# hongfz16/Garment4D

Hardware: AMD Instinct MI355X
Metric: point-cloud frames/s (FPS+ball_query+SA-MLP+LBS), B=8 N=8192 (higher is better)
Workload: dtype f32

## Files before the change

garment4d_amd/csrc/api.hip:

```cpp
#include <stdarg.h>
#include <stddef.h>
#include <stdlib.h>
#include <string.h>

#include "mlp_common.h"

namespace g4d {
static thread_local char g_err[512] = "";

void set_error(const char *fmt, ...) {
    va_list ap;
    va_start(ap, fmt);
    vsnprintf(g_err, sizeof(g_err), fmt, ap);
    va_end(ap);
}

static int g_contract = -1;

static int parse_contract(const char *e) {
    if (!e || !*e) return G4D_CONTRACT_NVCC;
    if (!strcmp(e, "0") || !strcmp(e, "off") || !strcmp(e, "none")) return G4D_CONTRACT_OFF;
    if (!strcmp(e, "2") || !strcmp(e, "chain") || !strcmp(e, "inner")) return G4D_CONTRACT_CHAIN;
    return G4D_CONTRACT_NVCC;
}

static thread_local int t_contract = -1;

int distance_contraction() {
    if (t_contract >= 0) return t_contract;
    int m = __atomic_load_n(&g_contract, __ATOMIC_RELAXED);
    if (m < 0) {
        m = parse_contract(getenv("G4D_DIST_CONTRACT"));
        __atomic_store_n(&g_contract, m, __ATOMIC_RELAXED);
    }
    return m;
}
}

namespace g4d {
namespace {
struct Tune { const char *key; long long value; int state; };
Tune g_tune[] = {{"sa_table_persistent", 0, 0}, {"sa_table_min_rows", 0, 0}, {"sa_table_128", 0, 0}, {"sa_table_oversub", 0, 0}, {"sa_table_dedup", 0, 0}, {"fp_table_persistent", 0, 0},
                 {"fp_table_min_rows", 0, 0}, {"gemm_tile", 0, 0}, {"gemm_tile_min_rows", 0, 0}, {"gemm_tile_min_cout", 0, 0}, {"gemm_tile_min_kpad", 0, 0}, {"fp_init_persistent", 0, 0}, {"fp_init_min_rows", 0, 0},
                 {"fp_head_bf16_persistent", 0, 0}, {"fp_head_bf16_min_rows", 0, 0}, {"sa_group_bf16_persistent", 0, 0}, {"sa_group_bf16_min_rows", 0, 0}};
}
struct ThreadTune { long long value; bool set; };
thread_local ThreadTune t_tune[sizeof(g_tune) / sizeof(g_tune[0])] = {};

long long tuning(const char *key, long long dflt) {
    int i = 0;
    for (Tune &t : g_tune) {
        const int slot = i++;
        if (strcmp(t.key, key)) continue;
        if (t_tune[slot].set) return t_tune[slot].value;
        int st = __atomic_load_n(&t.state, __ATOMIC_ACQUIRE);
        if (st == 0) {
            char env[64] = "G4D_";
            size_t n = 4;
            for (const char *c = key; *c && n + 1 < sizeof(env); ++c) env[n++] = (char)((*c >= 'a' && *c <= 'z') ? *c - 32 : *c);
            env[n] = 0;
            const char *e = getenv(env);
            const long long v = e && *e ? atoll(e) : dflt;
            int expect = 0;
            if (__atomic_compare_exchange_n(&t.state, &expect, 3, false, __ATOMIC_ACQ_REL, __ATOMIC_ACQUIRE)) {
                __atomic_store_n(&t.value, v, __ATOMIC_RELAXED);
                expect = 3;
                __atomic_compare_exchange_n(&t.state, &expect, 1, false, __ATOMIC_ACQ_REL, __ATOMIC_ACQUIRE);
                return v;
            }
            st = expect;
            if (st == 3) return v;
        }
        return __atomic_load_n(&t.value, __ATOMIC_RELAXED);
    }
    return dflt;
}
}

extern "C" int g4d_tuning_set(const char *key, long long value) {
    if (key)
        for (g4d::Tune &t : g4d::g_tune)
            if (!strcmp(t.key, key)) {
                __atomic_store_n(&t.value, value, __ATOMIC_RELAXED);
                __atomic_store_n(&t.state, 2, __ATOMIC_RELEASE);
                return G4D_OK;
            }
    g4d::set_error("g4d_tuning_set: unknown key '%s'", key ? key : "(null)");
    return G4D_EINVAL;
}

extern "C" int g4d_tuning_set_thread(const char *key, long long value, int set) {
    if (key) {
        int i = 0;
        for (g4d::Tune &t : g4d::g_tune) {
            const int slot = i++;
            if (!strcmp(t.key, key)) {
                g4d::t_tune[slot].value = value;
                g4d::t_tune[slot].set = set != 0;
                return G4D_OK;
            }
        }
    }
    g4d::set_error("g4d_tuning_set_thread: unknown key '%s'", key ? key : "(null)");
    return G4D_EINVAL;
}

extern "C" int g4d_version(void) { return 263;  }
extern "C" const char *g4d_last_error(void) { return g4d::g_err; }

extern "C" int g4d_get_distance_contraction(void) { return g4d::distance_contraction(); }
extern "C" int g4d_set_distance_contraction_thread(int mode) {
    const int prev = g4d::t_contract;
    if (mode < -1 || mode > G4D_CONTRACT_CHAIN) {
        g4d::set_error("g4d_set_distance_contraction_thread: mode %d is not -1 (no override) or one of G4D_CONTRACT_OFF/NVCC/CHAIN", mode);
        return -2;
    }
    g4d::t_contract = mode;
    return prev;
}

extern "C" int g4d_set_distance_contraction(int mode) {
    const int saved = g4d::t_contract;
    g4d::t_contract = -1;
    const int prev = g4d::distance_contraction();
    g4d::t_contract = saved;
    if (mode < G4D_CONTRACT_OFF || mode > G4D_CONTRACT_CHAIN) {
        g4d::set_error("g4d_set_distance_contraction: mode %d is not one of G4D_CONTRACT_OFF/NVCC/CHAIN", mode);
        return -1;
    }
    __atomic_store_n(&g4d::g_contract, mode, __ATOMIC_RELAXED);
    return prev;
}

namespace g4d {
struct CopySegs { float *dst[4]; const float *src[4]; long long n[4]; long long first_block[5]; };
__global__ void __launch_bounds__(256) copy_segments_kernel(const CopySegs c, int nseg) {
    int s = 0;
    while (s + 1 < nseg && (long long)blockIdx.x >= c.first_block[s + 1]) ++s;
    const long long i0 = ((long long)blockIdx.x - c.first_block[s]) * 1024 + threadIdx.x * 4;
    float *d = c.dst[s];
    const float *p = c.src[s];
    const long long n = c.n[s];
    if (i0 + 3 < n && ((reinterpret_cast<size_t>(d) | reinterpret_cast<size_t>(p)) & 15) == 0) {
        *reinterpret_cast<float4 *>(d + i0) = *reinterpret_cast<const float4 *>(p + i0);
    } else {
        for (int e = 0; e < 4; ++e)
            if (i0 + e < n) d[i0 + e] = p[i0 + e];
    }
}
}

extern "C" int g4d_copy_segments_f32(int nseg, float *const *dst, const float *const *src, const long long *nfloats, g4d_stream_t stream) {
    G4D_REQUIRE(nseg >= 0 && nseg <= 4 && (nseg == 0 || (dst && src && nfloats)), "g4d_copy_segments_f32: 0..4 segments");
    g4d::CopySegs c = {};
    long long blocks = 0;
    int k = 0;
    for (int i = 0; i < nseg; ++i) {
        G4D_REQUIRE(nfloats[i] >= 0 && (nfloats[i] == 0 || (dst[i] && src[i])), "g4d_copy_segments_f32: bad segment %d", i);
        if (nfloats[i] == 0) continue;
        c.dst[k] = dst[i]; c.src[k] = src[i]; c.n[k] = nfloats[i]; c.first_block[k] = blocks;
        blocks += (nfloats[i] + 1023) / 1024;
        ++k;
    }
    if (k == 0) return G4D_OK;
    c.first_block[k] = blocks;
    G4D_REQUIRE(blocks < (1ll << 31), "g4d_copy_segments_f32: too large");
    hipLaunchKernelGGL(g4d::copy_segments_kernel, dim3((unsigned)blocks), dim3(256), 0, reinterpret_cast<hipStream_t>(stream), c, k);
    return g4d::check_launch("g4d_copy_segments_f32");
}

namespace g4d {
static StackCall stack_call(const char *name, const g4d_mlp_args &a) {
    StackCall c = {};
    c.name = name; c.mode = a.mode; c.rows = a.rows;
    LinearArgs &in = c.in;
    in.K = a.K0; in.out = a.out; in.ldo = a.ldo; in.col0 = a.col0; in.pool = a.pool; in.S = a.S;
    in.X = a.X; in.ldx = a.ldx;
    in.xyz = a.xyz; in.new_xyz = a.new_xyz; in.feats = a.feats; in.idx = a.idx; in.N = a.N; in.P = a.P; in.C = a.C; in.use_xyz = a.use_xyz;
    in.known_feats = a.known_feats; in.skip = a.skip; in.dist2 = a.dist2; in.nn_idx = a.nn_idx; in.C2 = a.C2; in.C1 = a.C1; in.m = a.m; in.n = a.n;
    in.rowptr = a.rowptr; in.colidx = a.colidx; in.vals = a.vals; in.Vg = a.Vg;
    c.nlayers = a.nlayers; c.W = a.W; c.scale = a.scale; c.shift = a.shift; c.Kpad = a.Kpad; c.Cout = a.Cout; c.relu = a.relu;
    c.tap_layer = a.tap_layer; c.tap_out = a.tap_out; c.tap_ld = a.tap_ld; c.unknown_grid = a.unknown_grid;
    return c;
}

int stack_call_check(const StackCall &c, const StackRules &r) {
    const int S = c.in.S, pool = c.in.pool;
    G4D_REQUIRE(c.mode >= 0 && c.mode <= (r.csr ? LOAD_CSR : LOAD_INTERP), "%s: %s", c.name, r.bad_mode);
    if (r.max_layers) G4D_REQUIRE(c.nlayers >= 1 && c.nlayers <= r.max_layers, "%s: 1..%d layers", c.name, r.max_layers);
    G4D_REQUIRE(c.rows >= 0 && c.rows < r.max_rows && c.in.K > 0, "%s: bad sizes", c.name);
    if (c.rows == 0) return kEmptyLaunch;
    G4D_REQUIRE(has_layer_arrays(c), "%s: null pointer", c.name);
    if (!r.max_layers) G4D_REQUIRE(g4d_mlp_chain_supported(c.nlayers, c.Cout), "%s: unsupported layer widths (see g4d_mlp_chain_supported)", c.name);
    G4D_REQUIRE(pool >= 0 && pool <= 2, "%s: pool must be 0|1|2", c.name);
    if (pool) G4D_REQUIRE((S == 4 || S == 8 || S == 16 || S == 32 || S == 64) && c.rows % S == 0, "%s: pooling needs S in {4,8,16,32,64}", c.name);
    for (int l = 0; l < c.nlayers; ++l) {
        const void *const *Wl = c.W + (size_t)l * r.w_pieces;
        G4D_REQUIRE(Wl[0] && (r.w_pieces == 1 || (Wl[1] && Wl[2])) && c.scale[l] && c.shift[l] && c.Kpad[l] % r.kpad_multiple == 0 && c.Cout[l] > 0, "%s: bad layer %d", c.name, l);
    }
    G4D_REQUIRE(tap_layer_of(c) < c.nlayers - 1, "%s: tap must be a hidden layer", c.name);
    return G4D_OK;
}
}

extern "C" unsigned g4d_mlp_args_size(void) { return (unsigned)sizeof(g4d_mlp_args); }

extern "C" int g4d_mlp_run(int family, const g4d_mlp_args *args, g4d_stream_t stream) {
    using namespace g4d;
    G4D_REQUIRE(args, "g4d_mlp_run: null argument block");
    G4D_REQUIRE(args->version == G4D_MLP_ARGS_VERSION, "g4d_mlp_run: argument block version %u, this library speaks %d", args->version, G4D_MLP_ARGS_VERSION);
    G4D_REQUIRE(args->size >= 16 && args->size <= sizeof(g4d_mlp_args), "g4d_mlp_run: argument block of %u bytes, this library's is %u (a newer caller?)",
                args->size, (unsigned)sizeof(g4d_mlp_args));
    g4d_mlp_args a;
    memset(&a, 0, sizeof(a));
    memcpy(&a, args, args->size);
    if (args->size < offsetof(g4d_mlp_args, tap_layer) + sizeof(int)) a.tap_layer = -1;
    if (family != G4D_MLP_CHAIN_BF16) a.unknown_grid = nullptr;
    hipStream_t st = reinterpret_cast<hipStream_t>(stream);
    switch (family) {
        case G4D_MLP_STACK_F32: return mlp_stack_f32_run(stack_call("g4d_mlp_stack_f32", a), st);
        case G4D_MLP_STACK_BF16: return mlp_stack_bf16_run(stack_call("g4d_mlp_stack_bf16", a), st);
        case G4D_MLP_WAVE_F32: return mlp_wave_f32_run(stack_call("g4d_mlp_wave_f32", a), st);
        case G4D_MLP_CHAIN_F32: return mlp_chain_f32_run(stack_call("g4d_mlp_chain_f32", a), st);
        case G4D_MLP_CHAIN_BF16: return mlp_chain_bf16_run(stack_call("g4d_mlp_chain_bf16", a), st);
        case G4D_MLP_CHAIN_BF16X3: return mlp_chain_bf16x3_run(stack_call("g4d_mlp_chain_bf16x3", a), st);
    }
    set_error("g4d_mlp_run: unknown kernel family %d", family);
    return G4D_EINVAL;
}

#define G4D_MLP_LOADERS                                                                                                                       \
    int mode, long long rows, int K0,  const float *X, int ldx,                                                            \
     int N, int P, int S, int C, int use_xyz, const float *xyz, const float *new_xyz, const float *feats, const int *idx,        \
     int n, int m, int C2, int C1, const float *known_feats, const float *skip, const float *dist2, const int *nn_idx
#define G4D_MLP_LAYERS(WT)                                                                                                                    \
    int nlayers, const WT *const *W, const float *const *scale, const float *const *shift, const int *Kpad, const int *Cout, const int *relu, \
     int pool, float *out, int ldo, int col0
#define G4D_MLP_COMMON                                                                                                                        \
    mode, rows, K0, X, ldx, N, P, S, C, use_xyz, xyz, new_xyz, feats, idx, n, m, C2, C1, known_feats, skip, dist2, nn_idx, nlayers,         \
    reinterpret_cast<const void *const *>(W), scale, shift, Kpad, Cout, relu, pool, out, ldo, col0

static g4d_mlp_args pack_args(G4D_MLP_LOADERS, G4D_MLP_LAYERS(void), int tap_layer = -1, float *tap_out = nullptr, int tap_ld = 0) {
    g4d_mlp_args a;
    memset(&a, 0, sizeof(a));
    a.size = (unsigned)sizeof(a); a.version = G4D_MLP_ARGS_VERSION;
    a.mode = mode; a.rows = rows; a.K0 = K0; a.X = X; a.ldx = ldx;
    a.N = N; a.P = P; a.S = S; a.C = C; a.use_xyz = use_xyz; a.xyz = xyz; a.new_xyz = new_xyz; a.feats = feats; a.idx = idx;
    a.n = n; a.m = m; a.C2 = C2; a.C1 = C1; a.known_feats = known_feats; a.skip = skip; a.dist2 = dist2; a.nn_idx = nn_idx;
    a.nlayers = nlayers; a.W = W; a.scale = scale; a.shift = shift; a.Kpad = Kpad; a.Cout = Cout; a.relu = relu;
    a.pool = pool; a.out = out; a.ldo = ldo; a.col0 = col0; a.tap_layer = tap_layer; a.tap_out = tap_out; a.tap_ld = tap_ld;
    return a;
}

extern "C" int g4d_mlp_stack_f32(G4D_MLP_LOADERS,  int Vg, const int *rowptr, const int *colidx, const float *vals, G4D_MLP_LAYERS(float),
                                 int tap_layer, float *tap_out, int tap_ld, g4d_stream_t stream) {
    g4d_mlp_args a = pack_args(G4D_MLP_COMMON, tap_layer, tap_out, tap_ld);
    a.Vg = Vg; a.rowptr = rowptr; a.colidx = colidx; a.vals = vals;
    return g4d_mlp_run(G4D_MLP_STACK_F32, &a, stream);
}

extern "C" int g4d_mlp_stack_bf16(G4D_MLP_LOADERS,  int Vg, const int *rowptr, const int *colidx, const float *vals, G4D_MLP_LAYERS(unsigned short),
                                  int tap_layer, float *tap_out, int tap_ld, g4d_stream_t stream) {
    g4d_mlp_args a = pack_args(G4D_MLP_COMMON, tap_layer, tap_out, tap_ld);
    a.Vg = Vg; a.rowptr = rowptr; a.colidx = colidx; a.vals = vals;
    return g4d_mlp_run(G4D_MLP_STACK_BF16, &a, stream);
}

extern "C" int g4d_mlp_wave_f32(G4D_MLP_LOADERS,  int Vg, const int *rowptr, const int *colidx, const float *vals, G4D_MLP_LAYERS(float),
                                g4d_stream_t stream) {
    g4d_mlp_args a = pack_args(G4D_MLP_COMMON);
    a.Vg = Vg; a.rowptr = rowptr; a.colidx = colidx; a.vals = vals;
    return g4d_mlp_run(G4D_MLP_WAVE_F32, &a, stream);
}

extern "C" int g4d_mlp_chain_f32(G4D_MLP_LOADERS, G4D_MLP_LAYERS(float), int tap_layer, float *tap_out, int tap_ld, g4d_stream_t stream) {
    g4d_mlp_args a = pack_args(G4D_MLP_COMMON, tap_layer, tap_out, tap_ld);
    return g4d_mlp_run(G4D_MLP_CHAIN_F32, &a, stream);
}

extern "C" int g4d_mlp_chain_bf16(G4D_MLP_LOADERS, G4D_MLP_LAYERS(unsigned short), int tap_layer, float *tap_out, int tap_ld, g4d_stream_t stream) {
    g4d_mlp_args a = pack_args(G4D_MLP_COMMON, tap_layer, tap_out, tap_ld);
    return g4d_mlp_run(G4D_MLP_CHAIN_BF16, &a, stream);
}

extern "C" int g4d_mlp_chain_cells_bf16(G4D_MLP_LOADERS, G4D_MLP_LAYERS(unsigned short), int tap_layer, float *tap_out, int tap_ld, const void *unknown_grid,
                                        g4d_stream_t stream) {
    g4d_mlp_args a = pack_args(G4D_MLP_COMMON, tap_layer, tap_out, tap_ld);
    a.unknown_grid = unknown_grid;
    return g4d_mlp_run(G4D_MLP_CHAIN_BF16, &a, stream);
}

extern "C" int g4d_mlp_chain_bf16x3(G4D_MLP_LOADERS, G4D_MLP_LAYERS(unsigned short), int tap_layer, float *tap_out, int tap_ld, g4d_stream_t stream) {
    g4d_mlp_args a = pack_args(G4D_MLP_COMMON, tap_layer, tap_out, tap_ld);
    return g4d_mlp_run(G4D_MLP_CHAIN_BF16X3, &a, stream);
}
```

garment4d_amd/csrc/fps.hip:

```cpp
#include "g4d_common.h"

namespace g4d {

template <int U>
__device__ __host__ constexpr int brev_small(int v) {
    int r = 0;
    for (int bit = 1, rb = U >> 1; bit < U; bit <<= 1, rb >>= 1)
        if (v & bit) r |= rb;
    return r;
}

__device__ __forceinline__ float min_f32(float a, float b) {
    float r;
    asm("v_min_f32 %0, %1, %2" : "=v"(r) : "v"(a), "v"(b));
    return r;
}

struct FpsCand {
    float val;
    unsigned rank;
    int k;
    int pad;
};

__device__ __forceinline__ unsigned fps_rank(int k, int bs, int log2bs) {
    const unsigned c = (unsigned)k & (unsigned)(bs - 1);
    const unsigned q = (unsigned)k >> log2bs;
    const unsigned br = log2bs ? (__builtin_bitreverse32(c) >> (32 - log2bs)) : 0u;
    return (br << 16) | q;
}

template <int W>
__device__ __forceinline__ unsigned long long row_max_u64(unsigned long long key) {
#define G4D_STEP(CTRL)                                                                                       \
    {                                                                                                        \
        const unsigned lo = (unsigned)__builtin_amdgcn_update_dpp(0, (int)(unsigned)key, CTRL, 0xf, 0xf, true);        \
        const unsigned hi = (unsigned)__builtin_amdgcn_update_dpp(0, (int)(unsigned)(key >> 32), CTRL, 0xf, 0xf, true); \
        const unsigned long long o = ((unsigned long long)hi << 32) | lo;                                    \
        key = o > key ? o : key;                                                                             \
    }
    G4D_STEP(0x111)
    G4D_STEP(0x112)
    if constexpr (W >= 8) G4D_STEP(0x114)
    if constexpr (W >= 16) G4D_STEP(0x118)
#undef G4D_STEP
    return key;
}

__device__ __forceinline__ void wave_argmax(float best, int k, int bs, int log2bs, float &wval, int &wk, unsigned &wrank) {
    wval = wave_max_f32(best);
    const unsigned long long hit = __builtin_amdgcn_ballot_w64(best == wval);
    int lane;
    if (__builtin_popcountll(hit) == 1) {
        lane = __builtin_ctzll(hit);
        wk = __builtin_amdgcn_readlane(k, lane);
        wrank = fps_rank(wk, bs, log2bs);
    } else {
        const unsigned r = (best == wval) ? fps_rank(k, bs, log2bs) : 0xffffffffu;
        wrank = wave_min_u32(r);
        lane = __builtin_ctzll(__builtin_amdgcn_ballot_w64(r == wrank));
        wk = __builtin_amdgcn_readlane(k, lane);
    }
}

template <int W, int U, int Q, int FM>
__global__ void __launch_bounds__(64 * W) fps_reg_kernel(int n, int m, int bs, int log2bs, const float *__restrict__ xyz_all,
                                                        float *__restrict__ temp_all, int *__restrict__ idx_all, float *__restrict__ nx_all) {
    constexpr int T = 64 * W, P = U * Q;
    extern __shared__ __attribute__((aligned(16))) unsigned char smem_raw[];
    float *sx = reinterpret_cast<float *>(smem_raw + 2 * 16 * 16);
    float *sy = sx + n;
    float *sz = sy + n;
    int *spick = reinterpret_cast<int *>(sz + n);

    const int t = threadIdx.x;
    const float *xyz = xyz_all + (size_t)blockIdx.x * n * 3;
    float *temp = temp_all + (size_t)blockIdx.x * n;
    int *idx = idx_all + (size_t)blockIdx.x * m;
    float *nx = nx_all ? nx_all + (size_t)blockIdx.x * m * 3 : nullptr;

    float px[P], py[P], pz[P], md[P];
#pragma unroll
    for (int i = 0; i < P; ++i) {
        const int k = t + brev_small<U>(i / Q) * T + (i % Q) * bs;
        const bool ok = k < n;
        px[i] = ok ? xyz[k * 3 + 0] : 0.f;
        py[i] = ok ? xyz[k * 3 + 1] : 0.f;
        pz[i] = ok ? xyz[k * 3 + 2] : 0.f;
        md[i] = ok ? (temp_all ? temp[k] : 1e10f) : -2.f;
        if (ok) { sx[k] = px[i]; sy[k] = py[i]; sz[k] = pz[i]; }
    }
    if (t == 0) spick[0] = 0;
    __syncthreads();

    float x1 = sx[0], y1 = sy[0], z1 = sz[0];
    const int wave = t >> 6;
    for (int j = 1; j < m; ++j) {
        float best = -1.f;
        int bslot = 0;
#pragma unroll
        for (int i = 0; i < P; ++i) {
            const float dx = px[i] - x1, dy = py[i] - y1, dz = pz[i] - z1;
            const float d = dist2<FM>(dx, dy, dz);
            const float d2 = min_f32(d, md[i]);
            md[i] = d2;
            const bool gt = d2 > best;
            bslot = gt ? i : bslot;
            best = gt ? d2 : best;
        }
        int k;
        if constexpr (P == 1) k = t;
        else k = t + brev_small<U>(bslot / Q) * T + (bslot % Q) * bs;
        float wval; int wk; unsigned wrank;
        wave_argmax(best, k, bs, log2bs, wval, wk, wrank);
        int old;
        if constexpr (W == 1) {
            old = wk;
        } else {
            unsigned long long *buf = reinterpret_cast<unsigned long long *>(smem_raw) + (j & 1) * 16;
            if ((t & 63) == 0)
                buf[wave] = ((unsigned long long)__float_as_uint(fmaxf(wval, 0.f)) << 32) | (unsigned)(~wrank);
            __syncthreads();
            const unsigned long long key = row_max_u64<W>(buf[t & (W - 1)]);
            const unsigned rank = ~(unsigned)__builtin_amdgcn_readlane((int)(unsigned)key, W - 1);
            const unsigned c = log2bs ? (__builtin_bitreverse32(rank >> 16) >> (32 - log2bs)) : 0u;
            old = (int)(((rank & 0xffffu) << log2bs) | c);
        }
        x1 = sx[old]; y1 = sy[old]; z1 = sz[old];
        if (t == 0) spick[j] = old;
    }
    if constexpr (W > 1) __syncthreads();
    for (int j = t; j < m; j += T) {
        const int k = spick[j];
        idx[j] = k;
        if (nx) { nx[j * 3 + 0] = sx[k]; nx[j * 3 + 1] = sy[k]; nx[j * 3 + 2] = sz[k]; }
    }
    if (temp_all) {
#pragma unroll
        for (int i = 0; i < P; ++i) {
            const int k = t + brev_small<U>(i / Q) * T + (i % Q) * bs;
            if (k < n) temp[k] = md[i];
        }
    }
}

template <int UA, int UB, int FM>
__global__ void __launch_bounds__(256) fps_reg_pair_kernel(int m2, const float *__restrict__ xyz_all, int *__restrict__ idx1_all,
                                                          float *__restrict__ nx1_all, int *__restrict__ idx2_all, float *__restrict__ nx2_all) {
    constexpr int T = 256, W = 4, nA = T * UA, bsA = nA, m1 = 64 * UB, bsB = m1;
    constexpr int log2bsA = UA == 1 ? 8 : (UA == 2 ? 9 : 10), log2bsB = UB == 1 ? 6 : (UB == 2 ? 7 : (UB == 4 ? 8 : 9));
    extern __shared__ __attribute__((aligned(16))) unsigned char smem_raw[];
    float *sx = reinterpret_cast<float *>(smem_raw + 2 * 16 * 16);
    float *sy = sx + nA;
    float *sz = sy + nA;
    int *spick = reinterpret_cast<int *>(sz + nA);
    float *bx = reinterpret_cast<float *>(spick + m1);
    float *by = bx + m1;
    float *bz = by + m1;
    int *spick2 = reinterpret_cast<int *>(bz + m1);
    const int t = threadIdx.x;
    const float *xyz = xyz_all + (size_t)blockIdx.x * nA * 3;

    {
        float px[UA], py[UA], pz[UA], md[UA];
#pragma unroll
        for (int i = 0; i < UA; ++i) {
            const int k = t + brev_small<UA>(i) * T;
            px[i] = xyz[k * 3 + 0]; py[i] = xyz[k * 3 + 1]; pz[i] = xyz[k * 3 + 2];
            md[i] = 1e10f;
            sx[k] = px[i]; sy[k] = py[i]; sz[k] = pz[i];
        }
        if (t == 0) spick[0] = 0;
        __syncthreads();
        float x1 = sx[0], y1 = sy[0], z1 = sz[0];
        const int wave = t >> 6;
        for (int j = 1; j < m1; ++j) {
            float best = -1.f;
            int bslot = 0;
#pragma unroll
            for (int i = 0; i < UA; ++i) {
                const float dx = px[i] - x1, dy = py[i] - y1, dz = pz[i] - z1;
                const float d = dist2<FM>(dx, dy, dz);
                const float d2 = min_f32(d, md[i]);
                md[i] = d2;
                const bool gt = d2 > best;
                bslot = gt ? i : bslot;
                best = gt ? d2 : best;
            }
            const int k = UA == 1 ? t : t + brev_small<UA>(bslot) * T;
            float wval; int wk; unsigned wrank;
            wave_argmax(best, k, bsA, log2bsA, wval, wk, wrank);
            unsigned long long *buf = reinterpret_cast<unsigned long long *>(smem_raw) + (j & 1) * 16;
            if ((t & 63) == 0) buf[wave] = ((unsigned long long)__float_as_uint(fmaxf(wval, 0.f)) << 32) | (unsigned)(~wrank);
            __syncthreads();
            const unsigned long long key = row_max_u64<W>(buf[t & (W - 1)]);
            const unsigned rank = ~(unsigned)__builtin_amdgcn_readlane((int)(unsigned)key, W - 1);
            const unsigned c = __builtin_bitreverse32(rank >> 16) >> (32 - log2bsA);
            const int old = (int)(((rank & 0xffffu) << log2bsA) | c);
            x1 = sx[old]; y1 = sy[old]; z1 = sz[old];
            if (t == 0) spick[j] = old;
        }
        __syncthreads();
        int *idx = idx1_all + (size_t)blockIdx.x * m1;
        float *nx = nx1_all + (size_t)blockIdx.x * m1 * 3;
        for (int j = t; j < m1; j += T) {
            const int k = spick[j];
            idx[j] = k;
            const float x = sx[k], y = sy[k], z = sz[k];
            nx[j * 3 + 0] = x; nx[j * 3 + 1] = y; nx[j * 3 + 2] = z;
            bx[j] = x; by[j] = y; bz[j] = z;
        }
        __syncthreads();
    }
    if (t >= 64) return;
    {
        float px[UB], py[UB], pz[UB], md[UB];
#pragma unroll
        for (int i = 0; i < UB; ++i) {
            const int k = t + brev_small<UB>(i) * 64;
            px[i] = bx[k]; py[i] = by[k]; pz[i] = bz[k];
            md[i] = 1e10f;
        }
        if (t == 0) spick2[0] = 0;
        float x1 = bx[0], y1 = by[0], z1 = bz[0];
        for (int j = 1; j < m2; ++j) {
            float best = -1.f;
            int bslot = 0;
#pragma unroll
            for (int i = 0; i < UB; ++i) {
                const float dx = px[i] - x1, dy = py[i] - y1, dz = pz[i] - z1;
                const float d = dist2<FM>(dx, dy, dz);
                const float d2 = min_f32(d, md[i]);
                md[i] = d2;
                const bool gt = d2 > best;
                bslot = gt ? i : bslot;
                best = gt ? d2 : best;
            }
            const int k = UB == 1 ? t : t + brev_small<UB>(bslot) * 64;
            float wval; int wk; unsigned wrank;
            wave_argmax(best, k, bsB, log2bsB, wval, wk, wrank);
            const int old = wk;
            x1 = bx[old]; y1 = by[old]; z1 = bz[old];
            if (t == 0) spick2[j] = old;
        }
        __builtin_amdgcn_fence(__ATOMIC_RELEASE, "wavefront");
        __builtin_amdgcn_wave_barrier();
        __builtin_amdgcn_fence(__ATOMIC_ACQUIRE, "wavefront");
        int *idx = idx2_all + (size_t)blockIdx.x * m2;
        float *nx = nx2_all + (size_t)blockIdx.x * m2 * 3;
        for (int j = t; j < m2; j += 64) {
            const int k = spick2[j];
            idx[j] = k;
            nx[j * 3 + 0] = bx[k]; nx[j * 3 + 1] = by[k]; nx[j * 3 + 2] = bz[k];
        }
    }
}

template <int FM>
__global__ void __launch_bounds__(1024) fps_generic_kernel(int n, int m, int bs, int log2bs, const float *__restrict__ xyz_all,
                                                          float *__restrict__ temp_all, int *__restrict__ idx_all, float *__restrict__ nx_all) {
    constexpr int W = 16;
    __shared__ FpsCand slots[2][W];
    const int t = threadIdx.x;
    const float *xyz = xyz_all + (size_t)blockIdx.x * n * 3;
    float *temp = temp_all + (size_t)blockIdx.x * n;
    int *idx = idx_all + (size_t)blockIdx.x * m;
    float *nx = nx_all ? nx_all + (size_t)blockIdx.x * m * 3 : nullptr;
    if (t == 0) idx[0] = 0;
    int old = 0;
    const int wave = t >> 6;
    for (int j = 1; j <= m; ++j) {
        const float x1 = xyz[old * 3 + 0], y1 = xyz[old * 3 + 1], z1 = xyz[old * 3 + 2];
        if (t == 0 && nx) { nx[(j - 1) * 3 + 0] = x1; nx[(j - 1) * 3 + 1] = y1; nx[(j - 1) * 3 + 2] = z1; }
        if (j == m) break;
        float best = -1.f;
        int besti = 0;
        if (t < bs) {
            for (int k = t; k < n; k += bs) {
                const float dx = xyz[k * 3 + 0] - x1, dy = xyz[k * 3 + 1] - y1, dz = xyz[k * 3 + 2] - z1;
                const float d = dist2<FM>(dx, dy, dz);
                const float d2 = fminf(d, temp[k]);
                temp[k] = d2;
                const bool gt = d2 > best;
                besti = gt ? k : besti;
                best = gt ? d2 : best;
            }
        } else {
            best = -3.f;
        }
        float wval; int wk; unsigned wrank;
        {
            wval = wave_max_f32(best);
            const unsigned r = (best == wval) ? ((t < bs ? ((log2bs ? (__builtin_bitreverse32((unsigned)t) >> (32 - log2bs)) : 0u) << 16) : 0xffff0000u) |
                                                 (unsigned)(besti >> log2bs))
                                              : 0xffffffffu;
            wrank = wave_min_u32(r);
            const int lane = __builtin_ctzll(__builtin_amdgcn_ballot_w64(r == wrank));
            wk = __builtin_amdgcn_readlane(besti, lane);
        }
        FpsCand *buf = slots[j & 1];
        if ((t & 63) == 0) { FpsCand c; c.val = wval; c.rank = wrank; c.k = wk; c.pad = 0; buf[wave] = c; }
        __syncthreads();
        FpsCand bc = buf[0];
#pragma unroll
        for (int w = 1; w < W; ++w) {
            const FpsCand c = buf[w];
            const bool take = (c.val > bc.val) || (c.val == bc.val && c.rank < bc.rank);
            bc.val = take ? c.val : bc.val;
            bc.rank = take ? c.rank : bc.rank;
            bc.k = take ? c.k : bc.k;
        }
        old = __builtin_amdgcn_readfirstlane(bc.k);
        if (t == 0) idx[j] = old;
    }
}

static int ref_block_size(int work_size) {
    const int pow_2 = (int)(std::log((double)work_size) / std::log(2.0));
    int v = 1 << pow_2;
    if (v > 1024) v = 1024;
    if (v < 1) v = 1;
    return v;
}

template <int W, int U, int Q, int FM>
static int launch_reg_fm(int b, int n, int m, int bs, int log2bs, const float *xyz, float *temp, int *idx, float *nx, hipStream_t s) {
    const size_t lds = 2 * 16 * 16 + (size_t)n * 12 + (size_t)m * 4;
    auto kern = fps_reg_kernel<W, U, Q, FM>;
    static unsigned long long attr_done = 0;
    if (const int rc = ensure_dynamic_lds(reinterpret_cast<const void *>(kern), 160 * 1024 - 1024, attr_done, "g4d_fps_f32")) return rc;
    hipLaunchKernelGGL(kern, dim3(b), dim3(64 * W), lds, s, n, m, bs, log2bs, xyz, temp, idx, nx);
    return check_launch("g4d_fps_f32");
}

template <int W, int U, int Q>
static int launch_reg(int b, int n, int m, int bs, int log2bs, const float *xyz, float *temp, int *idx, float *nx, hipStream_t s) {
    G4D_WITH_FM(distance_contraction(), return (launch_reg_fm<W, U, Q, FM>(b, n, m, bs, log2bs, xyz, temp, idx, nx, s)))
    return G4D_OK;
}

int fps_bucket_dispatch(int b, int n, int m, int bs, int log2bs, const float *xyz, float *temp, int *idx, float *nx, hipStream_t s);
int fps_big_dispatch(int b, int n, int m, int bs, int log2bs, const float *xyz, float *temp, int *idx, float *nx, hipStream_t s);
int fps_bucket_grid_launch(int b, int n, int m, int bs, int log2bs, const float *xyz, int *idx, float *nx, float rmax, void *grid_ws, hipStream_t s);


static int g_fps_force_w = -1;

}

static int fps_impl(int b, int n, int m, const float *xyz, float *temp, int *idx, float *nx, g4d_stream_t stream) {
    using namespace g4d;
    G4D_REQUIRE(b >= 0 && n >= 0 && m >= 0, "g4d_fps_f32: negative size (b=%d n=%d m=%d)", b, n, m);
    if (b == 0 || m == 0) return G4D_OK;
    G4D_REQUIRE(n > 0, "g4d_fps_f32: n must be > 0 when m > 0");
    G4D_REQUIRE(xyz && idx, "g4d_fps_f32: null pointer");
    hipStream_t s = reinterpret_cast<hipStream_t>(stream);
    const int bs = ref_block_size(n);
    int log2bs = 0;
    while ((1 << log2bs) < bs) ++log2bs;
    const int q = (n + bs - 1) / bs;
    if (g_fps_force_w < 0) {
        const char *e = getenv("G4D_FPS_W");
        g_fps_force_w = e ? atoi(e) : 99;
    }
    const int force = g_fps_force_w;
    static const int use_bucket = getenv("G4D_FPS_BUCKET") ? atoi(getenv("G4D_FPS_BUCKET")) : 1;
    if (use_bucket && force > 16 && n > (use_bucket >= 2 ? 2048 : 4096) && n <= 8192) {
        const int rc = fps_bucket_dispatch(b, n, m, bs, log2bs, xyz, temp, idx, nx, s);
        if (rc >= 0) return rc;
    }
    static const int use_big = getenv("G4D_FPS_BIG") ? atoi(getenv("G4D_FPS_BIG")) : 1;
    const bool lds_ok = (size_t)n * 12 + (size_t)m * 4 + 512 <= 158 * 1024;
    if (use_big && force > 16 && n > 8192 && n <= 32768 && (use_big >= 2 || !(lds_ok && n <= 12800))) {
        const int rc = fps_big_dispatch(b, n, m, bs, log2bs, xyz, temp, idx, nx, s);
        if (rc >= 0) return rc;
    }
#define G4D_FPS_CASE(W, U, Q) return launch_reg<W, U, Q>(b, n, m, bs, log2bs, xyz, temp, idx, nx, s)
    if (lds_ok && force != 0 && bs >= 64) {
        const int qp = q <= 1 ? 1 : q <= 2 ? 2 : q <= 4 ? 4 : q <= 8 ? 8 : q <= 16 ? 16 : 0;
        const bool want_w1 = (force == 1) || (force > 16 && n <= 512);
        if (want_w1 && qp && (bs / 64) * qp <= 32) {
            const int u = bs / 64;
            if (u == 1 && qp == 1) G4D_FPS_CASE(1, 1, 1);
            if (u == 1 && qp == 2) G4D_FPS_CASE(1, 1, 2);
            if (u == 2 && qp == 1) G4D_FPS_CASE(1, 2, 1);
            if (u == 2 && qp == 2) G4D_FPS_CASE(1, 2, 2);
            if (u == 4 && qp == 1) G4D_FPS_CASE(1, 4, 1);
            if (u == 4 && qp == 2) G4D_FPS_CASE(1, 4, 2);
            if (u == 8 && qp == 1) G4D_FPS_CASE(1, 8, 1);
            if (u == 8 && qp == 2) G4D_FPS_CASE(1, 8, 2);
            if (u == 16 && qp == 1) G4D_FPS_CASE(1, 16, 1);
            if (u == 16 && qp == 2) G4D_FPS_CASE(1, 16, 2);
        }
        const int wsel = (force == 4 || force == 8 || force == 16) ? force : (n > 2048 ? 16 : 4);
        if (wsel == 16 && bs == 1024 && qp && qp <= 8) {
            if (qp == 1) G4D_FPS_CASE(16, 1, 1);
            if (qp == 2) G4D_FPS_CASE(16, 1, 2);
            if (qp == 4) G4D_FPS_CASE(16, 1, 4);
            if (qp == 8) G4D_FPS_CASE(16, 1, 8);
        }
        if (wsel >= 8 && bs >= 512 && qp && qp <= 8) {
            const int u = bs / 512;
            if (u == 1 && qp == 1) G4D_FPS_CASE(8, 1, 1);
            if (u == 1 && qp == 2) G4D_FPS_CASE(8, 1, 2);
            if (u == 2 && qp == 1) G4D_FPS_CASE(8, 2, 1);
            if (u == 2 && qp == 2) G4D_FPS_CASE(8, 2, 2);
            if (u == 2 && qp == 4) G4D_FPS_CASE(8, 2, 4);
            if (u == 2 && qp == 8) G4D_FPS_CASE(8, 2, 8);
        }
        if (bs >= 256 && qp) {
            const int u = bs / 256;
            if (u == 1 && qp == 1) G4D_FPS_CASE(4, 1, 1);
            if (u == 1 && qp == 2) G4D_FPS_CASE(4, 1, 2);
            if (u == 2 && qp == 1) G4D_FPS_CASE(4, 2, 1);
            if (u == 2 && qp == 2) G4D_FPS_CASE(4, 2, 2);
            if (u == 4 && qp == 1) G4D_FPS_CASE(4, 4, 1);
            if (u == 4 && qp == 2) G4D_FPS_CASE(4, 4, 2);
            if (u == 4 && qp == 4) G4D_FPS_CASE(4, 4, 4);
            if (u == 4 && qp == 8) G4D_FPS_CASE(4, 4, 8);
            if (u == 4 && qp == 16) G4D_FPS_CASE(4, 4, 16);
        }
        if (bs >= 64 && bs < 256 && qp && (bs / 64) * qp <= 32) {
            const int u = bs / 64;
            if (u == 1 && qp == 1) G4D_FPS_CASE(1, 1, 1);
            if (u == 1 && qp == 2) G4D_FPS_CASE(1, 1, 2);
            if (u == 2 && qp == 1) G4D_FPS_CASE(1, 2, 1);
            if (u == 2 && qp == 2) G4D_FPS_CASE(1, 2, 2);
        }
    }
#undef G4D_FPS_CASE
    G4D_REQUIRE(temp, "g4d_fps_f32: temp scratch (B,N) is required for this N (the scratch-free kernels cover 64 <= N <= 32768)");
    G4D_WITH_FM(distance_contraction(), hipLaunchKernelGGL(fps_generic_kernel<FM>, dim3(b), dim3(1024), 0, s, n, m, bs, log2bs, xyz, temp, idx, nx))
    return check_launch("g4d_fps_f32(generic)");
}

extern "C" int g4d_fps_f32(int b, int n, int m, const float *xyz, float *temp, int *idx, g4d_stream_t stream) {
    return fps_impl(b, n, m, xyz, temp, idx, nullptr, stream);
}

extern "C" int g4d_fps_gather_f32(int b, int n, int m, const float *xyz, float *temp, int *idx, float *new_xyz, g4d_stream_t stream) {
    G4D_REQUIRE(new_xyz || b == 0 || m == 0, "g4d_fps_gather_f32: new_xyz is NULL");
    return fps_impl(b, n, m, xyz, temp, idx, new_xyz, stream);
}

extern "C" int g4d_fps_gather_pair_supported(int n, int m1, int m2) { return n == 1024 && m1 == 256 && m2 >= 1 && m2 <= m1; }
extern "C" int g4d_fps_gather_pair_f32(int b, int n, int m1, int m2, const float *xyz, int *idx1, float *new_xyz1, int *idx2, float *new_xyz2,
                                       g4d_stream_t stream) {
    using namespace g4d;
    G4D_REQUIRE(b >= 0 && g4d_fps_gather_pair_supported(n, m1, m2), "g4d_fps_gather_pair_f32: unsupported shape (n=%d m1=%d m2=%d)", n, m1, m2);
    if (b == 0) return G4D_OK;
    G4D_REQUIRE(xyz && idx1 && new_xyz1 && idx2 && new_xyz2, "g4d_fps_gather_pair_f32: null pointer");
    const size_t lds = 2 * 16 * 16 + (size_t)n * 12 + (size_t)m1 * 16 + (size_t)m2 * 4;
    hipStream_t s = reinterpret_cast<hipStream_t>(stream);
    G4D_WITH_FM(distance_contraction(), hipLaunchKernelGGL((fps_reg_pair_kernel<4, 4, FM>), dim3(b), dim3(256), lds, s, m2, xyz, idx1, new_xyz1, idx2, new_xyz2))
    return check_launch("g4d_fps_gather_pair_f32");
}

extern "C" int g4d_ball_grid_build_f32(int b, int n, float rmax, const float *xyz, void *grid, g4d_stream_t stream);
extern "C" int g4d_fps_gather_grid_f32(int b, int n, int m, const float *xyz, int *idx, float *new_xyz, float rmax, void *grid, g4d_stream_t stream) {
    using namespace g4d;
    G4D_REQUIRE(b >= 0 && n > 0 && m > 0 && rmax > 0.f, "g4d_fps_gather_grid_f32: bad sizes");
    if (b == 0) return G4D_OK;
    G4D_REQUIRE(xyz && idx && new_xyz && grid, "g4d_fps_gather_grid_f32: null pointer");
    static const int merged = getenv("G4D_FPS_GRID_MERGED") ? atoi(getenv("G4D_FPS_GRID_MERGED")) : 1;
    static const int use_bucket = getenv("G4D_FPS_BUCKET") ? atoi(getenv("G4D_FPS_BUCKET")) : 1;
    if (merged && use_bucket && !getenv("G4D_FPS_W") && !getenv("G4D_FPS_BUCKET_W") && !getenv("G4D_FPS_DEAL")) {
        const int bs = ref_block_size(n);
        int log2bs = 0;
        while ((1 << log2bs) < bs) ++log2bs;
        const int rc = fps_bucket_grid_launch(b, n, m, bs, log2bs, xyz, idx, new_xyz, rmax, grid, reinterpret_cast<hipStream_t>(stream));
        if (rc >= 0) return rc;
    }
    if (const int rc = g4d_fps_gather_f32(b, n, m, xyz, nullptr, idx, new_xyz, stream)) return rc;
    return g4d_ball_grid_build_f32(b, n, rmax, xyz, grid, stream);
}
```

garment4d_amd/tuning.py:

```python
import contextlib
import contextvars
import dataclasses
import os
from typing import Mapping, Tuple


def _env_flag(name, default):
    return os.environ.get(name, "1" if default else "0") != "0"


def _env_int(name, default):
    return int(os.environ.get(name, str(default)))


NATIVE_KEYS = ("sa_table_persistent", "sa_table_min_rows", "sa_table_128", "sa_table_oversub", "sa_table_dedup", "fp_table_persistent", "fp_table_min_rows", "gemm_tile",
               "gemm_tile_min_rows", "gemm_tile_min_cout", "gemm_tile_min_kpad", "fp_init_persistent", "fp_init_min_rows",
               "fp_head_bf16_persistent", "fp_head_bf16_min_rows", "sa_group_bf16_persistent", "sa_group_bf16_min_rows")


@dataclasses.dataclass(frozen=True)
class Tuning:
    use_wave: bool = True
    use_stack: bool = True
    use_chain: bool = True
    stream_gemm: bool = True
    bf16_min_rows: int = 0
    overlap_sampling: bool = False
    lanes_sort: bool = False
    coherent_lanes: bool = False
    grid_min_n: int = 4096
    fps_pair: bool = True
    bq_multi: bool = True
    search_multi: bool = True
    three_nn_grid_min_m: int = 4096
    nn_cells: bool = True
    nn_multi: bool = True
    nn_prune: bool = True
    sa_xyz_pair: bool = True
    use_sa_xyz: bool = True
    sa_xyz_table: bool = True
    sa_table: bool = True
    fp_wide_fused: bool = False
    fp_cells: bool = True
    fp_table: bool = True
    fp_gemm_bf16: bool = True
    fp_gemm_bf16_min_rows: int = 8192
    fp_wide_table: bool = True
    dropin_fused: bool = True
    dropin_whole_model: bool = True
    use_pe_kernel: bool = True
    gcn_fuse_stack: bool = True
    gcn_autograd: bool = False
    refine_autograd: bool = False
    mgn_autograd: bool = False
    stage1_autograd: bool = False
    mlp_autograd: bool = False
    lbs_fused: bool = True
    lbs_mfma: bool = True
    lbs_one_launch: bool = True
    lbs_one_launch_max_b: int = 1 << 30
    nearest_cull: bool = True
    native: Tuple[Tuple[str, int], ...] = ()

    def replace(self, **kw) -> "Tuning":
        nat = kw.pop("native", None)
        if nat is not None:
            if isinstance(nat, Mapping):
                merged = dict(self.native)
                merged.update({str(k): int(v) for k, v in nat.items()})
                nat = tuple(sorted(merged.items()))
            else:
                nat = tuple((str(k), int(v)) for k, v in nat)
            for k, _ in nat:
                if k not in NATIVE_KEYS:
                    raise KeyError(f"unknown native tuning key '{k}' (include/g4d.h lists them)")
            kw["native"] = nat
        return dataclasses.replace(self, **kw)


def from_environment() -> Tuning:
    d = Tuning()
    return Tuning(
        use_wave=_env_flag("G4D_MLP_WAVE", d.use_wave), use_chain=_env_flag("G4D_MLP_CHAIN", d.use_chain), stream_gemm=_env_flag("G4D_GEMM_STREAM", d.stream_gemm),
        bf16_min_rows=_env_int("G4D_BF16_MIN_ROWS", d.bf16_min_rows), overlap_sampling=_env_flag("G4D_OVERLAP_SAMPLING", d.overlap_sampling),
        lanes_sort=_env_flag("G4D_BQ_LANES_SORT", d.lanes_sort), coherent_lanes=_env_flag("G4D_BQ_LANES", d.coherent_lanes),
        grid_min_n=_env_int("G4D_BQ_GRID_MIN_N", d.grid_min_n), fps_pair=_env_flag("G4D_FPS_PAIR", d.fps_pair), bq_multi=_env_flag("G4D_BQ_MULTI", d.bq_multi),
        search_multi=_env_flag("G4D_SEARCH_MULTI", d.search_multi), three_nn_grid_min_m=_env_int("G4D_NN_GRID_MIN_M", d.three_nn_grid_min_m),
        nn_cells=_env_flag("G4D_NN_CELLS", d.nn_cells), nn_multi=_env_flag("G4D_NN_MULTI", d.nn_multi), nn_prune=_env_flag("G4D_NN_PRUNE", d.nn_prune), sa_xyz_pair=_env_flag("G4D_SA_XYZ_PAIR", d.sa_xyz_pair),
        use_sa_xyz=_env_flag("G4D_SA_XYZ", d.use_sa_xyz), sa_xyz_table=_env_flag("G4D_SA_XYZ_TABLE", d.sa_xyz_table), sa_table=_env_flag("G4D_SA_TABLE", d.sa_table),
        fp_wide_fused=_env_flag("G4D_FP_WIDE_FUSED", d.fp_wide_fused), fp_cells=_env_flag("G4D_FP_CELLS", d.fp_cells), fp_table=_env_flag("G4D_FP_TABLE", d.fp_table),
        fp_gemm_bf16=_env_flag("G4D_FP_GEMM_BF16", d.fp_gemm_bf16), fp_gemm_bf16_min_rows=_env_int("G4D_FP_GEMM_BF16_MIN_ROWS", d.fp_gemm_bf16_min_rows),
        fp_wide_table=_env_flag("G4D_FP_WIDE_TABLE", d.fp_wide_table), gcn_fuse_stack=_env_flag("G4D_GCN_FUSED", d.gcn_fuse_stack), gcn_autograd=_env_flag("G4D_GCN_AUTOGRAD", d.gcn_autograd),
        refine_autograd=_env_flag("G4D_REFINE_AUTOGRAD", d.refine_autograd), mgn_autograd=_env_flag("G4D_MGN_AUTOGRAD", d.mgn_autograd),
        stage1_autograd=_env_flag("G4D_STAGE1_AUTOGRAD", d.stage1_autograd), mlp_autograd=_env_flag("G4D_MLP_AUTOGRAD", d.mlp_autograd),
        dropin_fused=_env_flag("G4D_DROPIN_FUSED", d.dropin_fused), dropin_whole_model=_env_flag("G4D_DROPIN_WHOLE", d.dropin_whole_model), lbs_mfma=_env_flag("G4D_LBS_MFMA", d.lbs_mfma), lbs_one_launch=_env_flag("G4D_LBS_ONE", d.lbs_one_launch),
        lbs_one_launch_max_b=_env_int("G4D_LBS_ONE_MAX_B", d.lbs_one_launch_max_b), nearest_cull=_env_flag("G4D_NEAREST_CULL", d.nearest_cull))


DEFAULT = from_environment()
_CURRENT = contextvars.ContextVar("g4d_tuning", default=DEFAULT)


def current() -> Tuning:
    return _CURRENT.get()


@contextlib.contextmanager
def use(t: Tuning):
    outer = _CURRENT.get()
    token = _CURRENT.set(t)
    touched = {k for k, _ in t.native} | {k for k, _ in outer.native}
    try:
        if touched:
            _apply_native(dict(t.native), touched)
        yield t
    finally:
        _CURRENT.reset(token)
        if touched:
            _apply_native(dict(outer.native), touched)


def _apply_native(values, keys):
    from . import _lib
    for k in keys:
        if k in values:
            _lib.call("g4d_tuning_set_thread", k.encode(), int(values[k]), 1)
        else:
            _lib.call("g4d_tuning_set_thread", k.encode(), 0, 0)
```

Before: 52240.

## Skip nested FPS when input prefix is already farthest-point ordered

Adds a device-side check that tests whether the first M input points already form a valid farthest-point-sampling order, which holds when the input is itself the output of an earlier FPS. If the check passes, the kernel writes the identity indices and copies the prefix coordinates instead of running the sequential M-iteration selection loop. It applies to the single-stage kernel for 1024→256 and 256→64 and to the paired kernel. If the check fails, the kernel falls back to the normal loop. The check adds an O(M²) verification pass with early exit, which is extra work whenever the property does not hold.

```diff
diff --git a/garment4d_amd/csrc/api.hip b/garment4d_amd/csrc/api.hip
--- a/garment4d_amd/csrc/api.hip
+++ b/garment4d_amd/csrc/api.hip
@@ -42,7 +42,7 @@
 struct Tune { const char *key; long long value; int state; };
 Tune g_tune[] = {{"sa_table_persistent", 0, 0}, {"sa_table_min_rows", 0, 0}, {"sa_table_128", 0, 0}, {"sa_table_oversub", 0, 0}, {"sa_table_dedup", 0, 0}, {"fp_table_persistent", 0, 0},
                  {"fp_table_min_rows", 0, 0}, {"gemm_tile", 0, 0}, {"gemm_tile_min_rows", 0, 0}, {"gemm_tile_min_cout", 0, 0}, {"gemm_tile_min_kpad", 0, 0}, {"fp_init_persistent", 0, 0}, {"fp_init_min_rows", 0, 0},
-                 {"fp_head_bf16_persistent", 0, 0}, {"fp_head_bf16_min_rows", 0, 0}, {"sa_group_bf16_persistent", 0, 0}, {"sa_group_bf16_min_rows", 0, 0}};
+                 {"fp_head_bf16_persistent", 0, 0}, {"fp_head_bf16_min_rows", 0, 0}, {"sa_group_bf16_persistent", 0, 0}, {"sa_group_bf16_min_rows", 0, 0}, {"fps_nested", 0, 0}};
 }
 struct ThreadTune { long long value; bool set; };
 thread_local ThreadTune t_tune[sizeof(g_tune) / sizeof(g_tune[0])] = {};
diff --git a/garment4d_amd/csrc/fps.hip b/garment4d_amd/csrc/fps.hip
--- a/garment4d_amd/csrc/fps.hip
+++ b/garment4d_amd/csrc/fps.hip
@@ -63,7 +63,85 @@
     }
 }
 
-template <int W, int U, int Q, int FM>
+
+__device__ __forceinline__ int fps_flag_hint(int *sflag) {
+    return __builtin_amdgcn_readfirstlane(__hip_atomic_load(sflag, __ATOMIC_RELAXED, __HIP_MEMORY_SCOPE_WORKGROUP));
+}
+
+template <int M, int P, int FM>
+__device__ __forceinline__ bool fps_is_prefix_ordered(int t, const float (&px)[P], const float (&py)[P], const float (&pz)[P], const float *sx,
+                                                      const float *sy, const float *sz, float *sval, int *sflag) {
+    constexpr int CH = 16;
+    static_assert(M % 64 == 0 && M >= 64, "one lane per k, whole waves");
+    bool bad;
+    {
+        const float x0 = sx[0], y0 = sy[0], z0 = sz[0];
+        const float v1 = min_f32(dist2<FM>(sx[1] - x0, sy[1] - y0, sz[1] - z0), 1e10f);
+        bad = !(v1 > 0.f);
+#pragma unroll
+        for (int i = 0; i < P; ++i) {
+            const float m = min_f32(dist2<FM>(px[i] - x0, py[i] - y0, pz[i] - z0), 1e10f);
+            bad |= i == 0 ? (!(m < v1) && t != 1) : !(m < v1);
+        }
+    }
+    if (!__builtin_amdgcn_ballot_w64(bad)) {
+        const float xk = px[0], yk = py[0], zk = pz[0];
+        const int iend = __builtin_amdgcn_readfirstlane(t | 63) + 1;
+        float v = 1e10f;
+        for (int i0 = 0; i0 < iend; i0 += CH) {
+            const int seen = fps_flag_hint(sflag);
+#pragma unroll
+            for (int u = 0; u < CH; ++u) {
+                const int i = i0 + u;
+                const float d = dist2<FM>(xk - sx[i], yk - sy[i], zk - sz[i]);
+                const float v2 = min_f32(d, v);
+                v = i < t ? v2 : v;
+            }
+            if (seen) break;
+        }
+        sval[t] = v;
+        const float inf = __builtin_inff();
+        bad = (t > 0 && !(v > 0.f)) || !(fabsf(xk) < inf && fabsf(yk) < inf && fabsf(zk) < inf);
+    }
+    if (__builtin_amdgcn_ballot_w64(bad) && (t & 63) == 0) *sflag = 1;
+    __syncthreads();
+    if (*sflag == 0) {
+        float mj[P];
+        unsigned long long badm = 0;
+        const int wbase = __builtin_amdgcn_readfirstlane(t & ~63);
+#pragma unroll
+        for (int i = 0; i < P; ++i) mj[i] = 1e10f;
+        auto step = [&](int s) {
+            const float xs = sx[s], ys = sy[s], zs = sz[s], v = sval[s + 1];
+            const unsigned rel = (unsigned)(s + 1 - wbase);
+            const unsigned long long winner = rel < 64u ? 1ull << rel : 0ull;
+#pragma unroll
+            for (int i = 0; i < P; ++i) {
+                const float d = dist2<FM>(px[i] - xs, py[i] - ys, pz[i] - zs);
+                mj[i] = min_f32(d, mj[i]);
+                const unsigned long long f = __builtin_amdgcn_ballot_w64(!(mj[i] < v));
+                badm |= i == 0 ? f & ~winner : f;
+            }
+        };
+        constexpr int FULL = (M - 1) / CH * CH;
+        int s = 0;
+        for (; s < FULL; s += CH) {
+            const int seen = fps_flag_hint(sflag);
+#pragma unroll
+            for (int u = 0; u < CH; ++u) step(s + u);
+            if (badm || seen) break;
+        }
+        if (s == FULL) {
+#pragma unroll
+            for (int u = 0; u < M - 1 - FULL; ++u) step(FULL + u);
+        }
+        if (badm && (t & 63) == 0) *sflag = 1;
+    }
+    __syncthreads();
+    return *sflag == 0;
+}
+
+template <int W, int U, int Q, int FM, bool NEST = false>
 __global__ void __launch_bounds__(64 * W) fps_reg_kernel(int n, int m, int bs, int log2bs, const float *__restrict__ xyz_all,
                                                         float *__restrict__ temp_all, int *__restrict__ idx_all, float *__restrict__ nx_all) {
     constexpr int T = 64 * W, P = U * Q;
@@ -90,8 +168,19 @@
         md[i] = ok ? (temp_all ? temp[k] : 1e10f) : -2.f;
         if (ok) { sx[k] = px[i]; sy[k] = py[i]; sz[k] = pz[i]; }
     }
+    int *sflag = reinterpret_cast<int *>(smem_raw + 256);
+    if (NEST && t == 0) *sflag = 0;
     if (t == 0) spick[0] = 0;
     __syncthreads();
+    if constexpr (NEST) {
+        static_assert(Q == 1, "slot 0 must be point t");
+        if (fps_is_prefix_ordered<T, P, FM>(t, px, py, pz, sx, sy, sz, reinterpret_cast<float *>(spick), sflag)) {
+            idx[t] = t;
+            if (nx) { nx[t * 3 + 0] = px[0]; nx[t * 3 + 1] = py[0]; nx[t * 3 + 2] = pz[0]; }
+            return;
+        }
+        if (t == 0) spick[0] = 0;
+    }
 
     float x1 = sx[0], y1 = sy[0], z1 = sz[0];
     const int wave = t >> 6;
@@ -145,7 +234,7 @@
 }
 
 template <int UA, int UB, int FM>
-__global__ void __launch_bounds__(256) fps_reg_pair_kernel(int m2, const float *__restrict__ xyz_all, int *__restrict__ idx1_all,
+__global__ void __launch_bounds__(256) fps_reg_pair_kernel(int m2, int nested, const float *__restrict__ xyz_all, int *__restrict__ idx1_all,
                                                           float *__restrict__ nx1_all, int *__restrict__ idx2_all, float *__restrict__ nx2_all) {
     constexpr int T = 256, W = 4, nA = T * UA, bsA = nA, m1 = 64 * UB, bsB = m1;
     constexpr int log2bsA = UA == 1 ? 8 : (UA == 2 ? 9 : 10), log2bsB = UB == 1 ? 6 : (UB == 2 ? 7 : (UB == 4 ? 8 : 9));
@@ -171,7 +260,22 @@
             sx[k] = px[i]; sy[k] = py[i]; sz[k] = pz[i];
         }
         if (t == 0) spick[0] = 0;
+        int *sflag = reinterpret_cast<int *>(smem_raw + 256);
+        if (t == 0) *sflag = 0;
         __syncthreads();
+        if constexpr (m1 == T) {
+            if (nested && fps_is_prefix_ordered<m1, UA, FM>(t, px, py, pz, sx, sy, sz, bx, sflag)) {
+                idx1_all[(size_t)blockIdx.x * m1 + t] = t;
+                float *nx = nx1_all + ((size_t)blockIdx.x * m1 + t) * 3;
+                nx[0] = px[0]; nx[1] = py[0]; nx[2] = pz[0];
+                if (t < m2) {
+                    idx2_all[(size_t)blockIdx.x * m2 + t] = t;
+                    float *nx2 = nx2_all + ((size_t)blockIdx.x * m2 + t) * 3;
+                    nx2[0] = px[0]; nx2[1] = py[0]; nx2[2] = pz[0];
+                }
+                return;
+            }
+        }
         float x1 = sx[0], y1 = sy[0], z1 = sz[0];
         const int wave = t >> 6;
         for (int j = 1; j < m1; ++j) {
@@ -323,10 +427,10 @@
     return v;
 }
 
-template <int W, int U, int Q, int FM>
+template <int W, int U, int Q, int FM, bool NEST = false>
 static int launch_reg_fm(int b, int n, int m, int bs, int log2bs, const float *xyz, float *temp, int *idx, float *nx, hipStream_t s) {
     const size_t lds = 2 * 16 * 16 + (size_t)n * 12 + (size_t)m * 4;
-    auto kern = fps_reg_kernel<W, U, Q, FM>;
+    auto kern = fps_reg_kernel<W, U, Q, FM, NEST>;
     static unsigned long long attr_done = 0;
     if (const int rc = ensure_dynamic_lds(reinterpret_cast<const void *>(kern), 160 * 1024 - 1024, attr_done, "g4d_fps_f32")) return rc;
     hipLaunchKernelGGL(kern, dim3(b), dim3(64 * W), lds, s, n, m, bs, log2bs, xyz, temp, idx, nx);
@@ -336,6 +440,12 @@
 template <int W, int U, int Q>
 static int launch_reg(int b, int n, int m, int bs, int log2bs, const float *xyz, float *temp, int *idx, float *nx, hipStream_t s) {
     G4D_WITH_FM(distance_contraction(), return (launch_reg_fm<W, U, Q, FM>(b, n, m, bs, log2bs, xyz, temp, idx, nx, s)))
+    return G4D_OK;
+}
+
+template <int W, int U>
+static int launch_reg_nested(int b, int n, int m, int bs, int log2bs, const float *xyz, int *idx, float *nx, hipStream_t s) {
+    G4D_WITH_FM(distance_contraction(), return (launch_reg_fm<W, U, 1, FM, true>(b, n, m, bs, log2bs, xyz, nullptr, idx, nx, s)))
     return G4D_OK;
 }
 
@@ -374,6 +484,10 @@
     if (use_big && force > 16 && n > 8192 && n <= 32768 && (use_big >= 2 || !(lds_ok && n <= 12800))) {
         const int rc = fps_big_dispatch(b, n, m, bs, log2bs, xyz, temp, idx, nx, s);
         if (rc >= 0) return rc;
+    }
+    if (!temp && force > 16 && tuning("fps_nested", 1)) {
+        if (n == 1024 && m == 256) return launch_reg_nested<4, 4>(b, n, m, bs, log2bs, xyz, idx, nx, s);
+        if (n == 256 && m == 64) return launch_reg_nested<1, 4>(b, n, m, bs, log2bs, xyz, idx, nx, s);
     }
 #define G4D_FPS_CASE(W, U, Q) return launch_reg<W, U, Q>(b, n, m, bs, log2bs, xyz, temp, idx, nx, s)
     if (lds_ok && force != 0 && bs >= 64) {
@@ -452,7 +566,8 @@
     G4D_REQUIRE(xyz && idx1 && new_xyz1 && idx2 && new_xyz2, "g4d_fps_gather_pair_f32: null pointer");
     const size_t lds = 2 * 16 * 16 + (size_t)n * 12 + (size_t)m1 * 16 + (size_t)m2 * 4;
     hipStream_t s = reinterpret_cast<hipStream_t>(stream);
-    G4D_WITH_FM(distance_contraction(), hipLaunchKernelGGL((fps_reg_pair_kernel<4, 4, FM>), dim3(b), dim3(256), lds, s, m2, xyz, idx1, new_xyz1, idx2, new_xyz2))
+    const int nested = tuning("fps_nested", 1) != 0;
+    G4D_WITH_FM(distance_contraction(), hipLaunchKernelGGL((fps_reg_pair_kernel<4, 4, FM>), dim3(b), dim3(256), lds, s, m2, nested, xyz, idx1, new_xyz1, idx2, new_xyz2))
     return check_launch("g4d_fps_gather_pair_f32");
 }
 
diff --git a/garment4d_amd/tuning.py b/garment4d_amd/tuning.py
--- a/garment4d_amd/tuning.py
+++ b/garment4d_amd/tuning.py
@@ -15,7 +15,7 @@
 
 NATIVE_KEYS = ("sa_table_persistent", "sa_table_min_rows", "sa_table_128", "sa_table_oversub", "sa_table_dedup", "fp_table_persistent", "fp_table_min_rows", "gemm_tile",
                "gemm_tile_min_rows", "gemm_tile_min_cout", "gemm_tile_min_kpad", "fp_init_persistent", "fp_init_min_rows",
-               "fp_head_bf16_persistent", "fp_head_bf16_min_rows", "sa_group_bf16_persistent", "sa_group_bf16_min_rows")
+               "fp_head_bf16_persistent", "fp_head_bf16_min_rows", "sa_group_bf16_persistent", "sa_group_bf16_min_rows", "fps_nested")
 
 
 @dataclasses.dataclass(frozen=True)
```

New measurement: 52860, median of 6. 1.01x the previous value.
